# stevengj/nlopt

Measured on NVIDIA H100. Metric: ccsa_dual_evals_per_sec, higher is better.
Workload: dtype f64

## Files before the change

### nlopt_b200/csrc/ccsa_kernels.cuh

```cuda
#pragma once

#include <cuda_runtime.h>

#include <cstdint>

#include "dual_mma.hpp"
#include "pair_math.cuh"

namespace nb200 {

constexpr int kBlock = 256;
constexpr int kWarps = kBlock / 32;
constexpr int kVirtualShards = 8;
constexpr int kMaxParamM = 16;
constexpr int kMaxNV = 3 + kMaxParamM;
constexpr int kWideMaxM = 2048;

__device__ __forceinline__ double mulx(double a, double b) { return __dmul_rn(a, b); }
__device__ __forceinline__ double addx(double a, double b) { return __dadd_rn(a, b); }
__device__ __forceinline__ double subx(double a, double b) { return __dsub_rn(a, b); }
__device__ __forceinline__ double divx(double a, double b) { return __ddiv_rn(a, b); }

__device__ __forceinline__ unsigned long long nb_globaltimer()
{
// ... 1811 lines not shown
            } else {
                xc.x = ccsaq_point<MAXM, true>(mu, vx.x, vlb.x, vub.x, vs.x, vg.x, Ga, acc);
                xc.y = ccsaq_point<MAXM, true>(mu, vx.y, vlb.y, vub.y, vs.y, vg.y, Gb, acc);
            }
            if (store) st_stream(reinterpret_cast<double2 *>(a.xcur) + mt.p + sub * 32 + lane, xc);
        }
        if (mt.flags & 2u) {
            warp_fold<NV>(acc);
            double *srec = s_rec[parity];
            if (lane == 0) {
#pragma unroll
                for (int k = 0; k < NV; ++k) srec[sub * NV + k] = acc[k];
            }
            asm volatile("bar.sync 1, %0;" ::"r"(32 * kGroupWarps) : "memory");
            parity ^= 1;
            if (sub == 0) put_group_record<NV>(srec, a.grouptags, ngroups, mt.gl, sa.tag0 | my_gen, lane);
            NB_TR(if (sub == 0 && lane == 0 && my_gen < kTraceGens) { const unsigned long long t = nb_globaltimer(); unsigned long long *r = sa.trace + 16 * my_gen;
                      atomicMax(r + 3, ~t); atomicMax(r + 4, t); atomicAdd(r + 8, t - tr_s0); atomicAdd(r + 9, 1ull); tr_last = t; })
        }
    }
    if (threadIdx.x == 0) {
        s_stop = 1;
        while (!s_prod_done) __nanosleep(20);
        __threadfence_block();
        const unsigned long long issued = s_issued;
        unsigned long long done = consumed + 1;
        if (++st == STAGES) { st = 0; phase ^= 1u; }
        for (; done < issued; ++done) {
            mbar_wait(&s_full[st], phase);
            if (++st == STAGES) { st = 0; phase ^= 1u; }
        }
    }
    asm volatile("bar.sync 1, %0;" ::"r"(32 * kGroupWarps) : "memory");
}

constexpr int kPenaltyRowsPerLaunch = 16;
struct PenaltyCoefs {
    double c[kPenaltyRowsPerLaunch];
    int row[kPenaltyRowsPerLaunch];
    int count;
};
__global__ void __launch_bounds__(kBlock) penalty_axpy_kernel(double *__restrict__ g, const double *__restrict__ rows,
                                                               unsigned long long ld, unsigned long long n_local,
                                                               const __grid_constant__ PenaltyCoefs pc)
{
    const unsigned long long stride = (unsigned long long) gridDim.x * blockDim.x;
    for (unsigned long long j = (unsigned long long) blockIdx.x * blockDim.x + threadIdx.x; j < n_local; j += stride) {
        double v = g[j];
        for (int k = 0; k < pc.count; ++k) v = addx(v, mulx(pc.c[k], rows[(unsigned long long) pc.row[k] * ld + j]));
        g[j] = v;
    }
}

__global__ void __launch_bounds__(kBlock) negate_kernel(double *__restrict__ g, unsigned long long n_local)
{
    constexpr unsigned long long kSign = 0x8000000000000000ull;
    const unsigned long long pairs = n_local >> 1, stride = (unsigned long long) gridDim.x * blockDim.x;
    const unsigned long long t = (unsigned long long) blockIdx.x * blockDim.x + threadIdx.x;
    ulonglong2 *g2 = reinterpret_cast<ulonglong2 *>(g);
    for (unsigned long long p = t; p < pairs; p += stride) {
        ulonglong2 v = g2[p];
        v.x ^= kSign;
        v.y ^= kSign;
        g2[p] = v;
    }
    if ((n_local & 1) && t == 0) {
        unsigned long long *tail = reinterpret_cast<unsigned long long *>(g) + (n_local - 1);
        *tail ^= kSign;
    }
}

__global__ void publish_kernel(const double *all_vsums , int nv, int nvp, volatile double *out_host,
                               volatile unsigned long long *flag_host, unsigned long long seq)
{
    for (int k = threadIdx.x; k < nv; k += blockDim.x) {
        double s = all_vsums[k];
        for (int v = 1; v < kVirtualShards; ++v) s = addx(s, all_vsums[v * nvp + k]);
        out_host[k] = s;
    }
    __threadfence_system();
    __syncthreads();
    if (threadIdx.x == 0) {
        *flag_host = seq;
        __threadfence_system();
    }
}

constexpr int kBoxHaloLeft = 20, kBoxHaloRight = 21;
struct HaloArgs {
    double *x;
    unsigned long long n_local;
    unsigned long long right_cell;
    double *box[8];
    int rank, world;
    unsigned long long seq;
};
__global__ void halo_exchange_kernel(const __grid_constant__ HaloArgs a)
{
    const int lane = threadIdx.x;
    const int buf = (int) (a.seq & 1ull);
    const bool left = a.rank > 0, right = a.rank + 1 < a.world;
    if (lane == 0 && left)
        box_put(a.box[a.rank - 1] + 2ull * ((unsigned long long) buf * 8 * kBoxStride + kBoxHaloRight), a.x[0], a.seq);
    if (lane == 1 && right)
        box_put(a.box[a.rank + 1] + 2ull * ((unsigned long long) buf * 8 * kBoxStride + kBoxHaloLeft), a.x[a.n_local - 1], a.seq);
    if ((lane == 0 && left) || (lane == 1 && right)) {
        const double *mine = a.box[a.rank] + 2ull * ((unsigned long long) buf * 8 * kBoxStride + (lane == 0 ? kBoxHaloLeft : kBoxHaloRight));
        const unsigned long long t0 = nb_globaltimer();
        double v;
        bool ok;
        while (!(ok = box_get(mine, a.seq, &v)))
            if (nb_globaltimer() - t0 > 10000000000ull) break;
        if (!ok) v = __longlong_as_double(0x7ff8000000000000ll);
        if (lane == 0) a.x[-1] = v; else a.x[a.right_cell] = v;
    }
}
__global__ void halo_apply_kernel(double *x, unsigned long long right_cell, const double *edges, int rank, int world)
{
    if (threadIdx.x == 0 && rank > 0) x[-1] = edges[2 * (rank - 1) + 1];
    if (threadIdx.x == 1 && rank + 1 < world) x[right_cell] = edges[2 * (rank + 1)];
}
__global__ void halo_pack_kernel(const double *x, unsigned long long n_local, double *edges, int rank)
{
    if (threadIdx.x == 0) { edges[2 * rank] = x[0]; edges[2 * rank + 1] = x[n_local - 1]; }
}

__global__ void fill_kernel(double *dst, double value, unsigned long long n_local)
{
    for (unsigned long long j = blockIdx.x * (unsigned long long) blockDim.x + threadIdx.x; j < n_local;
         j += (unsigned long long) gridDim.x * blockDim.x)
        dst[j] = value;
}

__device__ __forceinline__ bool dev_isinf(double v) { return fabs(v) >= HUGE_VAL * 0.99 || isinf(v); }

__global__ void sigma_init_kernel(double *sigma, const double *lb, const double *ub, const double *sigma_init,
                                  double sigma_min, unsigned long long n_local, unsigned short *sidx)
{
    for (unsigned long long j = blockIdx.x * (unsigned long long) blockDim.x + threadIdx.x; j < n_local;
         j += (unsigned long long) gridDim.x * blockDim.x) {
        double s;
        if (sigma_init && sigma_init[j] > 0) s = sigma_init[j];
        else if (dev_isinf(ub[j]) || dev_isinf(lb[j])) s = 1.0;
        else s = mulx(0.5, subx(ub[j], lb[j]));
        sigma[j] = s > sigma_min ? s : sigma_min;
        if (sidx) sidx[j] = 1;
    }
}

struct EndOuterArgs {
    const double *xcur;
    double *xprev, *xprevprev, *sigma;
    const double *lb, *ub;
    const double *w;
    const double *xtol_abs;
    unsigned long long n_local, nchunks, chunk0;
    unsigned nseg_total, seg0, segs_per_vshard, local_vshards;
    double *partials, *vsums;
    unsigned *tickets;
    double *out_dev;
    volatile double *out_host;
    volatile unsigned long long *flag_host;
    unsigned long long seq;
    int publish_host, nvp;
    int update_sigma;
    double kappa;
    double sigma_min;
    unsigned short *sidx;
    const unsigned short *next;
    const double *pal;
};

__global__ void __launch_bounds__(kBlock) end_outer_kernel(const __grid_constant__ EndOuterArgs a)
{
    constexpr int NV = 4;
    __shared__ double s_red[kWarps * NV];
    __shared__ int s_flag;
    const unsigned seg = a.seg0 + blockIdx.x;
    unsigned long long p_lo, p_hi;
    group_pairs(a.nchunks, a.nseg_total, a.chunk0, seg, &p_lo, &p_hi);
    double acc[NV] = {0.0, 0.0, 0.0, 0.0};
    for (unsigned long long p = p_lo + threadIdx.x; p < p_hi; p += kBlock) {
#pragma unroll
        for (int h = 0; h < 2; ++h) {
            const unsigned long long j = 2 * p + h;
            if (j >= a.n_local) break;
            const double xc = a.xcur[j], xp = a.xprev[j];
            const double d = fabs(subx(xc, xp));
            if (a.w) {
                acc[0] = addx(acc[0], mulx(a.w[j], d));
                acc[1] = addx(acc[1], mulx(a.w[j], fabs(xc)));
            } else {
                acc[0] = addx(acc[0], d);
                acc[1] = addx(acc[1], fabs(xc));
            }
            if (a.xtol_abs && d >= a.xtol_abs[j]) acc[2] = addx(acc[2], 1.0);
            if (a.update_sigma) {
                const double xpp = a.xprevprev[j];
                const double osc = mulx(subx(xc, xp), subx(xp, xpp));
                const int br = osc < 0 ? 0 : (osc > 0 ? 1 : 2);
                const double s0 = a.sigma[j];
                double s = mulx(s0, br == 0 ? 0.7 : (br == 1 ? 1.2 : 1.0));
                const double lo = a.lb[j], hi = a.ub[j];
                if (!dev_isinf(hi) && !dev_isinf(lo)) {
                    const double range = subx(hi, lo);
                    const double top = mulx(10.0, range), bot = mulx(a.kappa, range);
                    s = s < top ? s : top;
                    s = s > bot ? s : bot;
                }
                s = s > a.sigma_min ? s : a.sigma_min;
                a.sigma[j] = s;
                if (a.sidx) {
                    const unsigned short i0 = a.sidx[j], t = a.next[3u * i0 + br];
                    a.sidx[j] = t;
                    if (__double_as_longlong(__ldg(a.pal + i0)) != __double_as_longlong(s0) ||
                        __double_as_longlong(__ldg(a.pal + t)) != __double_as_longlong(s))
                        acc[3] = addx(acc[3], 1.0);
                }
            }
            if (a.xprevprev) a.xprevprev[j] = xp;
            a.xprev[j] = xc;
        }
    }
    block_reduce_to<NV>(acc, s_red, a.partials + (unsigned long long) blockIdx.x * a.nvp);
    const unsigned vs_local = blockIdx.x / a.segs_per_vshard;
    if (!is_last_arrival(a.tickets + vs_local, a.segs_per_vshard, &s_flag)) return;
    acc[0] = acc[1] = acc[2] = acc[3] = 0.0;
    {
        const double *base = a.partials + (unsigned long long) vs_local * a.segs_per_vshard * a.nvp;
        for (unsigned sgi = threadIdx.x; sgi < a.segs_per_vshard; sgi += kBlock)
#pragma unroll
            for (int k = 0; k < NV; ++k) acc[k] = addx(acc[k], __ldcg(base + (unsigned long long) sgi * a.nvp + k));
    }
    block_reduce_to<NV>(acc, s_red, a.vsums + (unsigned long long) vs_local * a.nvp);
    if (!is_last_arrival(a.tickets + a.local_vshards, a.local_vshards, &s_flag)) return;
    if (threadIdx.x < NV) {
        if (a.publish_host) {
            double s = __ldcg(a.vsums + threadIdx.x);
            for (unsigned v = 1; v < a.local_vshards; ++v) s = addx(s, __ldcg(a.vsums + (unsigned long long) v * a.nvp + threadIdx.x));
            a.out_host[threadIdx.x] = s;
            __threadfence_system();
        } else {
            const unsigned v0 = a.seg0 / a.segs_per_vshard;
            for (unsigned v = 0; v < a.local_vshards; ++v)
                a.out_dev[(unsigned long long) (v0 + v) * a.nvp + threadIdx.x] = __ldcg(a.vsums + (unsigned long long) v * a.nvp + threadIdx.x);
        }
    }
    __syncthreads();
    if (threadIdx.x == 0) {
        for (unsigned v = 0; v <= a.local_vshards; ++v) a.tickets[v] = 0;
        if (a.publish_host) {
            *a.flag_host = a.seq;
            __threadfence_system();
        }
    }
}

}
```

### nlopt_b200/csrc/device_backend.cu

```cuda
#include "device_backend.hpp"

#include <chrono>
#include <cmath>
#include <cstdio>
#include <cstdlib>
#include <cstring>
#include <map>
#include <memory>
#include <mutex>
#include <string>
#include <vector>

#include "bounds_kernels.cuh"
#include "ccsa_kernels.cuh"
#include "comm.hpp"
#include "dual_mma.hpp"
#include "nlopt_object.hpp"
#include "synth.cuh"
#include "terms_kernels.cuh"

namespace nb200 {

namespace {

// ... 1328 lines not shown
    const bool tma_auto = solve_tma_ < 0 && scalar_bounds_ && (maxm == 4 || (maxm == 1 && operand_bytes <= ((size_t) 80 << 20)));
    size_t smem = 0;
    int block = 256;
    SolveKernel fn = nullptr;
    bool sb = false, si = false;
    if ((solve_tma_ > 0 || tma_auto) && full && !use_pol && (maxm == 1 || maxm == 2 || maxm == 4)) {
        sb = scalar_bounds_;
        si = sidx_valid_ && maxm == 4;
        const int bm = si ? kSigmaIndex : sb ? kScalarBounds : kBoundArrays;
        fn = variant_ == kMMA ? pick_solve_tma_kernel1<0>(bm, maxm, &smem) : pick_solve_tma_kernel1<1>(bm, maxm, &smem);
        block = kTmaBlock;
        NB_CUDA(cudaFuncSetAttribute((const void *) fn, cudaFuncAttributeMaxDynamicSharedMemorySize, (int) smem));
    } else if (solve_async_ >= 2 && !use_pol && maxm <= 8) {
        const int stages = solve_async_ >= 3 ? 3 : 2;
        fn = variant_ == kMMA ? pick_solve_async_kernel2<0>(maxm, full, stages) : pick_solve_async_kernel2<1>(maxm, full, stages);
        smem = (size_t) stages * (5 + (size_t) maxm) * kChunkBytes;
        NB_CUDA(cudaFuncSetAttribute((const void *) fn, cudaFuncAttributeMaxDynamicSharedMemorySize, (int) smem));
    } else {
        const bool roomy = solve_minb_ == 2 || (solve_minb_ != 3 && (long long) geo_.nseg_local + 1 <= 2ll * sm_count_);
        sb = scalar_bounds_ && !use_pol;
        fn = variant_ == kMMA ? pick_solve_kernel2<0>(maxm, full, use_pol, sb, roomy) : pick_solve_kernel2<1>(maxm, full, use_pol, sb, roomy);
    }
    int per_sm = 0;
    NB_CUDA(cudaOccupancyMaxActiveBlocksPerMultiprocessor(&per_sm, fn, block, smem));
    if (per_sm < 1) return fail("dual_solve_kernel does not fit on an SM");
    long long grid = (long long) per_sm * sm_count_;
    if (grid > (long long) geo_.nseg_local + 1) grid = (long long) geo_.nseg_local + 1;
    if (grid < 2) return fail("dual_solve_kernel needs two co-resident CTAs");

    NB_CUDA(cudaMemsetAsync(solve_state_, 0, offsetof(SolveState, pub), stream_));
    cudaEvent_t e0 = nullptr, e1 = nullptr;
    if (time_kernels_) {
        if (ev_used_ + 2 > ev_pool_.size()) {
            if (ev_pool_.size() >= 8192) drain_events();
            else
                for (int k = 0; k < 512; ++k) { cudaEvent_t e; cudaEventCreate(&e); ev_pool_.push_back(e); }
        }
        e0 = ev_pool_[ev_used_++];
        e1 = ev_pool_[ev_used_++];
        cudaEventRecord(e0, stream_);
    }
    void *params[] = {&sa};
    {
        cudaError_t le = cudaLaunchCooperativeKernel((const void *) fn, dim3((unsigned) grid), dim3((unsigned) block), params, smem, stream_);
        if (le != cudaSuccess) {
            cudaGetLastError();
            fused_solve_ok_ = false;
            if (ev_used_ >= 2 && time_kernels_) ev_used_ -= 2;
            return fail("cooperative launch of dual_solve_kernel", le);
        }
    }
    if (time_kernels_) cudaEventRecord(e1, stream_);
    ++stats_->kernel_launches;
    cand_in_x_ = false;
    ++x_epoch_;
    if (!wait_flag()) return false;
#ifdef NB200_TRACE
    if (const char *tf = std::getenv("NLOPT_B200_TRACE_FILE")) {
        static std::vector<unsigned long long> h(16 * kTraceGens);
        cudaStreamSynchronize(stream_);
        cudaMemcpy(h.data(), trace_buf, h.size() * sizeof(unsigned long long), cudaMemcpyDeviceToHost);
        std::string tfn = tf;
        if (Comm::instance().active()) tfn += ".r" + std::to_string(Comm::instance().rank);
        if (FILE *f = std::fopen(tfn.c_str(), "a")) {
            const unsigned long long t00 = ~h[1];
            std::fprintf(f, "solve n_local=%llu m=%u grid=%lld groups=%u cta_start_spread_ns=%llu first_publish_ns=%llu\n", (unsigned long long) geo_.n_local, m_, grid,
                         geo_.nseg_local, h[2] - t00, h[16] - t00);
            for (int g = 1; g < kTraceGens && h[16 * g]; ++g) {
                const unsigned long long *r = &h[16 * g];
                const unsigned long long p = r[0];
                std::fprintf(f, "  gen %d lastrec[%lld..%lld] parked[%lld..%lld] seen[%lld..%lld] recs[%lld..%lld] rank_done %lld totals %lld machine %lld next_pub %lld | mean_group_sweep %llu ns x %llu\n", g,
                             r[11] ? (long long) (~r[10] - p) : 0ll, r[11] ? (long long) (r[11] - p) : 0ll,
                             r[12] ? (long long) (~r[13] - p) : 0ll, r[12] ? (long long) (r[12] - p) : 0ll,
                             (long long) (~r[1] - p), (long long) (r[2] - p), (long long) (~r[3] - p), (long long) (r[4] - p),
                             (long long) (r[5] - p), (long long) (r[6] - p), (long long) (r[7] - p),
                             (long long) (h[16 * (g + 1)] ? h[16 * (g + 1)] - p : 0), r[9] ? r[8] / r[9] : 0ull, r[9]);
            }
            std::fclose(f);
        }
    }
#endif
    const long gens = (long) res_host_[kResCounts + 2];
    *ret = (int) res_host_[kResCounts + 1];
    *nevals = (long) res_host_[kResCounts];
    if (Comm::instance().active() && gens > 0) Comm::instance().advance_seq((unsigned long long) gens);
    if (*ret == kRetInvalid) return true;
    if (*ret == kRetFailure) return fail("the cross-rank exchange inside the dual solve timed out");
    count_operand_bytes(gens, sb, si, true);
    out->val = res_host_[0];
    out->gval = res_host_[1];
    out->wval = res_host_[2];
    for (unsigned i = 0; i < m_; ++i) {
        out->gc[i] = res_host_[3 + i];
        y[i] = res_host_[kResY + i];
    }
    return true;
}

void DeviceBackend::drain_events()
{
    if (!ev_used_) return;
    cudaStreamSynchronize(stream_);
    double ms = 0;
    for (size_t i = 0; i + 1 < ev_used_; i += 2) {
        float t = 0;
        if (cudaEventElapsedTime(&t, ev_pool_[i], ev_pool_[i + 1]) == cudaSuccess) ms += t;
    }
    stats_->seconds_dual_kernel += ms * 1e-3;
    ev_used_ = 0;
}

bool DeviceBackend::time_dual(const double *y, const DualScalars &sc, bool materialize, int iters, double *ms_avg)
{
    cudaEvent_t e0, e1;
    NB_CUDA(cudaEventCreate(&e0));
    NB_CUDA(cudaEventCreate(&e1));
    NB_CUDA(cudaEventRecord(e0, stream_));
    for (int it = 0; it < iters; ++it)
        if (!launch_dual(y, sc, materialize, false)) return false;
    NB_CUDA(cudaEventRecord(e1, stream_));
    NB_CUDA(cudaStreamSynchronize(stream_));
    float ms = 0;
    NB_CUDA(cudaEventElapsedTime(&ms, e0, e1));
    cudaEventDestroy(e0);
    cudaEventDestroy(e1);
    if (materialize) cand_in_x_ = false;
    *ms_avg = (double) ms / iters;
    return true;
}


void DeviceBackend::accept_candidate()
{
    std::swap(x_, xcur_);
    std::swap(g_, gcur_);
    std::swap(G_, Gcur_);
    cand_in_x_ = true;
    if (h_x_slot_ == (int) kCandidate && h_x_epoch_ == x_epoch_) h_x_slot_ = (int) kBase;
    if (h_xs_slot_ == (int) kCandidate && h_xs_epoch_ == x_epoch_) h_xs_slot_ = (int) kBase;
}

bool DeviceBackend::first_outer()
{
    NB_CUDA(cudaMemcpyAsync(xprev_, xcur_view(), geo_.ld * sizeof(double), cudaMemcpyDeviceToDevice, stream_));
    return true;
}

bool DeviceBackend::end_outer(unsigned k, double sigma_min, double *dnorm, double *xnorm, bool *all_below_abs)
{
    EndOuterArgs a;
    std::memset(&a, 0, sizeof a);
    a.xcur = xcur_view();
    a.xprev = xprev_; a.xprevprev = xprevprev_; a.sigma = sigma_;
    a.lb = lb_; a.ub = ub_;
    a.update_sigma = k > 1;
    a.kappa = variant_ == kMMA ? 0.01 : 1e-8;
    a.sigma_min = sigma_min;
    if (a.update_sigma && sidx_valid_) {
        sidx_valid_ = sigma_min == sidx_sigma_min_ && palette_.step();
        if (sidx_valid_ && !upload_palette()) return false;
        if (sidx_valid_) { a.sidx = sidx_; a.next = next_; a.pal = pal_; }
    }
    if (!end_outer_pass(a, dnorm, xnorm, all_below_abs)) return false;
    if (out_host_[3] != 0.0) {
        stats_->sigma_index_mismatches += (long long) out_host_[3];
        sidx_valid_ = false;
    }
    stats_->sigma_palette = sidx_valid_ ? (long long) palette_.val.size() : 0;
    return true;
}

bool DeviceBackend::end_outer_pass(EndOuterArgs &a, double *dnorm, double *xnorm, bool *all_below_abs)
{
    a.w = w_dev_; a.xtol_abs = xtol_abs_dev_;
    a.n_local = geo_.n_local; a.nchunks = geo_.nchunks; a.chunk0 = geo_.chunk0;
    a.nseg_total = geo_.S; a.seg0 = geo_.seg0; a.segs_per_vshard = geo_.P; a.local_vshards = geo_.local_vshards;
    a.partials = partials_; a.vsums = vsums_; a.tickets = tickets_; a.out_dev = out_dev_;
    a.out_host = out_host_; a.flag_host = flag_host_;
    a.seq = seq_ = Comm::instance().active() ? Comm::instance().next_seq() : seq_ + 1;
    a.publish_host = Comm::instance().active() ? 0 : 1;
    a.nvp = kEndNvp;
    end_outer_kernel<<<(int) geo_.nseg_local, kBlock, 0, stream_>>>(a);
    ++stats_->kernel_launches;
    NB_CUDA(cudaGetLastError());
    if (!a.publish_host) {
        if (Comm::instance().all_gather_inplace(out_dev_, (size_t) geo_.local_vshards * kEndNvp, stream_, &err_)) return false;
        publish_kernel<<<1, 32, 0, stream_>>>(out_dev_, 4, kEndNvp, out_host_, flag_host_, a.seq);
        ++stats_->kernel_launches;
        NB_CUDA(cudaGetLastError());
    }
    if (!wait_flag()) return false;
    *dnorm = out_host_[0];
    *xnorm = out_host_[1];
    *all_below_abs = out_host_[2] == 0.0;
    return true;
}

bool DeviceBackend::stop_x_keep(double *dnorm, double *xnorm, bool *all_below_abs)
{
    EndOuterArgs a;
    std::memset(&a, 0, sizeof a);
    a.xcur = x_;
    a.xprev = xprev_;
    return end_outer_pass(a, dnorm, xnorm, all_below_abs);
}

int DeviceBackend::ranks() const { return Comm::instance().active() ? Comm::instance().world : 1; }

bool DeviceBackend::fetch_x(double *x_out)
{
    drain_events();
    if (cfg_.values_only) {
        NB_CUDA(cudaMemcpyAsync(x_out, xprev_, geo_.n_local * sizeof(double), cfg_.x_dev ? cudaMemcpyDeviceToDevice : cudaMemcpyDeviceToHost, stream_));
        NB_CUDA(cudaStreamSynchronize(stream_));
        if (!cfg_.x_dev) stats_->d2h_bytes += geo_.n_local * sizeof(double);
        return true;
    }
    if (cfg_.x_dev && x_out == cfg_.x_dev) {
        NB_CUDA(cudaMemcpyAsync(x_out, x_, geo_.n_local * sizeof(double), cudaMemcpyDeviceToDevice, stream_));
        NB_CUDA(cudaStreamSynchronize(stream_));
        return true;
    }
    Comm &comm = Comm::instance();
    if (!comm.active()) {
        NB_CUDA(cudaMemcpyAsync(x_out, x_, geo_.n_local * sizeof(double), cudaMemcpyDeviceToHost, stream_));
        NB_CUDA(cudaStreamSynchronize(stream_));
        stats_->d2h_bytes += geo_.n_local * sizeof(double);
        return true;
    }
    if (!h_x_) NB_CUDA(cached_host_alloc(&h_x_, (size_t) geo_.n * sizeof(double)));
    if (!xfull_dev_) NB_CUDA(cached_malloc(&xfull_dev_, (size_t) comm.world * shard_cap_ * sizeof(double)));
    h_x_slot_ = -1;
    if (!host_x_for(kBase)) return false;
    std::memcpy(x_out, h_x_view_, (size_t) geo_.n * sizeof(double));
    return true;
}


double *DeviceBackend::array(const char *which)
{
    const std::string w = which;
    if (w == "x") return x_;
    if (w == "xcur") return xcur_view();
    if (w == "xprev") return xprev_;
    if (w == "xprevprev") return xprevprev_;
    if (w == "lb") return lb_;
    if (w == "ub") return ub_;
    if (w == "sigma") return sigma_;
    if (w == "grad_f") return g_;
    if (w == "grad_f_cur") return gcur_;
    return nullptr;
}

bool DeviceBackend::upload(const char *which, const double *host)
{
    double *dst = array(which);
    if (std::string(which) == "xcur") { dst = xcur_; cand_in_x_ = false; }
    if (!dst) return fail(std::string("unknown array ") + which);
    if (dst == sigma_) sidx_valid_ = false;
    NB_CUDA(cudaMemcpyAsync(dst, host + geo_.j0, geo_.n_local * sizeof(double), cudaMemcpyHostToDevice, stream_));
    NB_CUDA(cudaStreamSynchronize(stream_));
    return true;
}

bool DeviceBackend::upload_grad_c(const double *host)
{
    if (!m_) return true;
    NB_CUDA(cudaMemcpy2DAsync(G_, geo_.ld * sizeof(double), host + geo_.j0, (size_t) geo_.n * sizeof(double),
                              geo_.n_local * sizeof(double), m_, cudaMemcpyHostToDevice, stream_));
    NB_CUDA(cudaStreamSynchronize(stream_));
    return true;
}

bool DeviceBackend::download(const char *which, double *host)
{
    const std::string w = which;
    if (w == "grad_c") {
        if (!m_) return true;
        NB_CUDA(cudaMemcpy2DAsync(host + geo_.j0, (size_t) geo_.n * sizeof(double), G_, geo_.ld * sizeof(double),
                                  geo_.n_local * sizeof(double), m_, cudaMemcpyDeviceToHost, stream_));
        NB_CUDA(cudaStreamSynchronize(stream_));
        return true;
    }
    double *src = array(which);
    if (!src) return fail(std::string("unknown array ") + which);
    NB_CUDA(cudaMemcpyAsync(host + geo_.j0, src, geo_.n_local * sizeof(double), cudaMemcpyDeviceToHost, stream_));
    NB_CUDA(cudaStreamSynchronize(stream_));
    return true;
}

bool DeviceBackend::fill_synthetic(unsigned long long seed)
{
    SynthArgs a;
    a.x = x_; a.lb = lb_; a.ub = ub_; a.sigma = sigma_; a.g = g_; a.G = G_;
    a.ld = geo_.ld; a.n_local = geo_.n_local; a.j0 = geo_.j0; a.seed = seed; a.m = (int) m_;
    synth_fill_kernel<<<grid_for(geo_.n_local, sm_count_), kBlock, 0, stream_>>>(a);
    NB_CUDA(cudaGetLastError());
    NB_CUDA(cudaStreamSynchronize(stream_));
    cand_in_x_ = true;
    return true;
}

bool DeviceBackend::configure(const char *key, long long value)
{
    const std::string k = key;
    if (k == "time_kernels") { time_kernels_ = value != 0; return true; }
    if (k == "kernel_cfg") { kernel_cfg_ = (int) value; return true; }
    if (k == "ctas_per_sm") { ctas_per_sm_ = (int) value; return true; }
    if (k == "fused_solve") { fused_solve_ok_ = value != 0; return true; }
    if (k == "solve_tma") { solve_tma_ = (int) value; return true; }
    if (k == "solve_async") { solve_async_ = (int) value; return true; }
    if (k == "solve_minb") { solve_minb_ = (int) value; return true; }
    if (k == "l2_keep_mb") {
        l2_keep_bytes_ = value <= 0 ? 0 : (size_t) value << 20;
        int maxp = 0;
        if (cudaDeviceGetAttribute(&maxp, cudaDevAttrMaxPersistingL2CacheSize, device_) == cudaSuccess && maxp > 0) {
            size_t want = l2_keep_bytes_ < (size_t) maxp ? l2_keep_bytes_ : (size_t) maxp;
            cudaDeviceSetLimit(cudaLimitPersistingL2CacheSize, want);
            cudaGetLastError();
        }
        return true;
    }
    if (k == "pmax" || k == "target_chunks" || k == "fill_div" || k == "group_base" || k == "geometry_rule" || k == "group_min_chunks") {
        if (value < 1 && k != "geometry_rule") return fail("bad value");
        if (k == "pmax") pmax_ = (unsigned) value;
        else if (k == "target_chunks") target_chunks_ = (unsigned) value;
        else if (k == "group_base") Geometry::group_base() = (unsigned) value;
        else if (k == "group_min_chunks") Geometry::min_group_chunks() = (unsigned) value;
        else if (k == "geometry_rule") Geometry::rule() = (int) value;
        else Geometry::fill_div() = (unsigned) value;
        if (pool_) {
            Geometry g2 = Geometry::make(geo_.n, geo_.world, geo_.rank, target_chunks_, pmax_);
            if (g2.ld != geo_.ld || g2.j0 != geo_.j0)
                return fail("changing the segment geometry of a sharded, allocated problem is not supported");
            geo_ = g2;
            return alloc_workspace();
        }
        return true;
    }
    return fail(std::string("unknown key ") + key);
}

long long DeviceBackend::query(const char *key) const
{
    const std::string k = key;
    if (k == "kernel_ns") {
        const_cast<DeviceBackend *>(this)->drain_events();
        return (long long) (stats_->seconds_dual_kernel * 1e9);
    }
    if (k == "segments") return geo_.S;
    if (k == "segments_local") return geo_.nseg_local;
    if (k == "P") return geo_.P;
    if (k == "n_local") return (long long) geo_.n_local;
    if (k == "j0") return (long long) geo_.j0;
    if (k == "ld") return (long long) geo_.ld;
    if (k == "launches") return stats_->kernel_launches;
    if (k == "maxm") return pick_maxm((int) m_);
// ... 399 lines not shown
```

### nlopt_b200/csrc/device_backend.hpp

```cpp
#pragma once

#include <cuda_runtime.h>

#include <string>
#include <vector>

#include "backend_factory.hpp"
#include "geometry.hpp"
#include "sigma_palette.hpp"

#ifndef NB200_SIGMA_INDEX_MIN_MB
#define NB200_SIGMA_INDEX_MIN_MB 50
#endif

namespace nb200 {

class DeviceBackend : public Backend {
public:
    DeviceBackend();
    ~DeviceBackend() override;

    bool setup(const BackendConfig &cfg);
    bool setup_raw(Variant v, unsigned n, unsigned m);

    unsigned n() const override { return (unsigned) geo_.n; }
    unsigned m() const override { return m_; }
    unsigned num_constraint_objects() const override { return (unsigned) cfg_.constraints.size(); }
    unsigned constraint_dim(unsigned ic) const override { return cfg_.constraints[ic].m; }
    bool init_sigma(double sigma_min) override;
    bool eval_objective(Slot slot, bool want_grad, double *value) override;
    bool eval_constraint(Slot slot, unsigned ic, unsigned row0, bool want_grad, double *values) override;
    bool finish_evals(double *fvalue, double *cvalues) override;
    bool agree_any(bool local) override;
    bool enqueue_df2(const FuncSpec &fs, Slot slot, double *grad_dst, unsigned index);
    bool reduce_terms(const FuncSpec &fs, const double *xs, double *grad_dst, double *vsums);
    bool ensure_halo(Slot slot);
    bool eval_sharded(const FuncSpec &fs, Slot slot, double *grad_dst, unsigned index, double *value);
    bool eval_user_objective(Slot slot, bool want_grad, double *value);
    bool negate_gradient(double *g);
    bool push_rows_to(double *dst, unsigned rows, const double *host_grad);
    bool eval_penalty_objective(Slot slot, bool want_grad, double *value);
    bool dual_eval(const double *y, const DualScalars &sc, bool materialize, DualSums *out) override;
    bool supports_dual_solve() const override;
    bool dual_solve(double *y, const double *lo, const double *hi, const double *stop6, const DualScalars &sc, DualSums *out,
                    int *ret, long *nevals) override;
    void accept_candidate() override;
    bool first_outer() override;
    bool end_outer(unsigned k, double sigma_min, double *dnorm, double *xnorm, bool *all_below_abs) override;
    bool fetch_x(double *x_out) override;
    double *point_device() override { return cfg_.values_only ? x_ : nullptr; }
    void point_moved() override { ++x_epoch_; }
    bool stop_x_keep(double *dnorm, double *xnorm, bool *all_below_abs) override;
    int ranks() const override;
    const std::string &error() const override { return err_; }
    double seconds_in_callbacks() const override { return cb_seconds_; }

    bool upload(const char *which, const double *host);
    bool upload_grad_c(const double *host_rowmajor_m_by_n);
    bool download(const char *which, double *host);
    bool fill_synthetic(unsigned long long seed);
    bool sigma_init_from(const double *sigma_init_host, double sigma_min);
    bool set_norm_arrays(const double *x_weights_host, const double *xtol_abs_host);
    bool time_dual(const double *y, const DualScalars &sc, bool materialize, int iters, double *ms_avg);
    bool configure(const char *key, long long value) override;
    long long query(const char *key) const;
    const Geometry &geometry() const { return geo_; }
    bool is_mma() const { return variant_ == kMMA; }

private:
    bool fail(const char *what, cudaError_t e);
    bool fail(const std::string &what);
    bool alloc_state();
    void free_state();
    bool alloc_workspace();
    double *array(const char *which);
    double *xcur_view() { return cand_in_x_ ? x_ : xcur_; }
    void fill_dual_args(struct DualArgs &a, const double *y, const DualScalars &sc);
    bool launch_dual(const double *y, const DualScalars &sc, bool store, bool wait);
    bool end_outer_pass(struct EndOuterArgs &a, double *dnorm, double *xnorm, bool *all_below_abs);
    unsigned l2_keep_mask() const;
    void count_operand_bytes(long long evals, bool sb, bool si, bool store);
    bool upload_palette();
    bool sigma_index_runs() const;
    bool wait_flag();
    bool host_x_for(Slot slot);
    bool push_grad_rows(Slot slot, int row0, unsigned rows, bool is_objective, const double *host_grad);
    double *staging(unsigned rows);
    struct Owned { void *p; size_t bytes; bool pinned; };
    std::vector<Owned> owned_;
    bool small_dev(void **p, size_t bytes);
    bool small_pinned(void **p, size_t bytes);
    void release_small(void *p);

    BackendConfig cfg_;
    Variant variant_ = kMMA;
    unsigned m_ = 0;
    Geometry geo_;
    unsigned target_chunks_ = kDefaultTargetChunks, pmax_ = kDefaultPmax;
    int device_ = 0;
    int sm_count_ = 132, ctas_per_sm_ = 0;
    void *solve_state_ = nullptr;
    double *res_host_ = nullptr;
    double *grouptags_ = nullptr;
    unsigned long long eval_tag_ = 0;
    double *wide_dev_ = nullptr;
    std::vector<double> wide_host_;
    size_t l2_keep_bytes_ = 0;
    int solve_tma_ = -1;
    int solve_async_ = 0;
    int solve_minb_ = 0;
    size_t out_rec_ = 0;
    unsigned long long solve_launch_id_ = 0;
    bool fused_solve_ok_ = true;
    bool scalar_bounds_ = false;
    double lb_u_ = 0.0, ub_u_ = 0.0;
    bool sidx_valid_ = false;
    unsigned short *sidx_ = nullptr, *next_ = nullptr;
    double *pal_ = nullptr;
    double *pal_pinned_ = nullptr;
    unsigned short *next_pinned_ = nullptr;
    SigmaPalette palette_;
    size_t pal_uploaded_ = 0, rows_uploaded_ = 0;
    double sidx_sigma_min_ = 0.0;
    int kernel_cfg_ = -1;

    double *pool_ = nullptr;
    size_t pool_bytes_ = 0;
    double *x_ = nullptr, *xcur_ = nullptr, *xprev_ = nullptr, *xprevprev_ = nullptr, *lb_ = nullptr, *ub_ = nullptr,
           *sigma_ = nullptr, *g_ = nullptr, *gcur_ = nullptr, *G_ = nullptr, *Gcur_ = nullptr;
    double *w_dev_ = nullptr, *xtol_abs_dev_ = nullptr;
    bool cand_in_x_ = true;

    double *partials_ = nullptr, *vsums_ = nullptr, *out_dev_ = nullptr;
    unsigned *tickets_ = nullptr;
    double *out_host_ = nullptr;
    unsigned long long *flag_host_ = nullptr;
    unsigned long long seq_ = 0;
    int nvp_ = 24;

    double *h_x_ = nullptr;
    double *h_x_view_ = nullptr;
    double *h_grad_[2] = {nullptr, nullptr};
    size_t h_grad_cap_ = 0;
    int h_grad_next_ = 0;
    cudaEvent_t h_grad_done_[2] = {nullptr, nullptr};
    double *h_xs_ = nullptr, *h_gs_[2] = {nullptr, nullptr};
    cudaEvent_t h_gs_done_[2] = {nullptr, nullptr};
    int h_gs_next_ = 0, h_xs_slot_ = -1;
    unsigned long long h_xs_epoch_ = 0;
    double *xfull_dev_ = nullptr;
    double *pen_rows_ = nullptr;
    unsigned pen_total_ = 0;
    double *scalar_dev_ = nullptr;
    std::vector<double> pend_val_;
    std::vector<char> pend_set_;
    bool pend_any_ = false;
    size_t scalar_cap_ = 0;
    double *vs2_dev_ = nullptr, *vs2_host_ = nullptr;
    size_t vs2_cap_ = 0;
    std::vector<const FuncSpec *> pend2_;
    bool pend2_any_ = false;
    unsigned terms_rows_ = 0;
    double *terms_ = nullptr, *terms_part_ = nullptr;
    nlopt_b200_shard shard_{};
    double *halo_edges_ = nullptr;
    const double *halo_ptr_ = nullptr;
    unsigned long long halo_epoch_ = 0;
    size_t shard_cap_ = 0;
    unsigned long long x_epoch_ = 1, h_x_epoch_ = 0;
    int h_x_slot_ = -1;

    cudaStream_t stream_ = nullptr, copy_stream_ = nullptr;

    bool time_kernels_ = false;
    std::vector<cudaEvent_t> ev_pool_;
    size_t ev_used_ = 0;
    void drain_events();

    std::string err_;
    double cb_seconds_ = 0;
    nlopt_b200_stats local_stats_{};
    nlopt_b200_stats *stats_ = &local_stats_;
    unsigned max_cdim_ = 1;
};

void release_cached_blocks();

}
```

Before: 5716.

## Vectorize end_outer loads/stores, use scalar bounds, rotate xprev buffers

The end-of-outer-iteration kernel now loads and stores element pairs with double2/ushort2 vector accesses. When bounds are uniform it uses scalar bound values instead of reading the lb/ub arrays. It also writes xcur into the xprevprev buffer and swaps the xprev/xprevprev pointers on the host, which saves one array write per element. This cuts global memory traffic in a bandwidth-bound kernel. The risks are alignment assumptions for the vector accesses and correctness of the buffer rotation when xprevprev is null or the first pass differs.

After: 5717, median of 6. Within noise of the previous version (+0.0%).

```diff
diff --git a/nlopt_b200/csrc/ccsa_kernels.cuh b/nlopt_b200/csrc/ccsa_kernels.cuh
--- a/nlopt_b200/csrc/ccsa_kernels.cuh
+++ b/nlopt_b200/csrc/ccsa_kernels.cuh
@@ -1987,6 +1987,8 @@
     const double *xcur;
     double *xprev, *xprevprev, *sigma;
     const double *lb, *ub;
+    double lb_u, ub_u;
+    int rotate;
     const double *w;
     const double *xtol_abs;
     unsigned long long n_local, nchunks, chunk0;
@@ -2006,6 +2008,29 @@
     const double *pal;
 };
 
+template <class T, class T2>
+__device__ __forceinline__ void ld_pair(T (&v)[2], const T *row, unsigned long long j, bool full)
+{
+    if (full) {
+        const T2 t = *reinterpret_cast<const T2 *>(row + j);
+        v[0] = t.x;
+        v[1] = t.y;
+    } else
+        v[0] = row[j];
+}
+template <class T, class T2>
+__device__ __forceinline__ void st_pair(T *row, unsigned long long j, const T (&v)[2], bool full)
+{
+    if (full) {
+        T2 t;
+        t.x = v[0];
+        t.y = v[1];
+        *reinterpret_cast<T2 *>(row + j) = t;
+    } else
+        row[j] = v[0];
+}
+
+template <bool SB = false>
 __global__ void __launch_bounds__(kBlock) end_outer_kernel(const __grid_constant__ EndOuterArgs a)
 {
     constexpr int NV = 4;
@@ -2016,45 +2041,65 @@
     group_pairs(a.nchunks, a.nseg_total, a.chunk0, seg, &p_lo, &p_hi);
     double acc[NV] = {0.0, 0.0, 0.0, 0.0};
     for (unsigned long long p = p_lo + threadIdx.x; p < p_hi; p += kBlock) {
+        const unsigned long long j0 = 2 * p;
+        if (j0 >= a.n_local) break;
+        const bool full = j0 + 1 < a.n_local;
+        const int nh = full ? 2 : 1;
+        double xc[2] = {0.0, 0.0}, xp[2] = {0.0, 0.0}, xpp[2] = {0.0, 0.0}, s0[2] = {0.0, 0.0};
+        double lo[2] = {a.lb_u, a.lb_u}, hi[2] = {a.ub_u, a.ub_u}, s[2] = {0.0, 0.0};
+        unsigned short i0[2] = {0, 0}, t[2] = {0, 0};
+        ld_pair<double, double2>(xc, a.xcur, j0, full);
+        ld_pair<double, double2>(xp, a.xprev, j0, full);
+        if (a.update_sigma) {
+            ld_pair<double, double2>(xpp, a.xprevprev, j0, full);
+            ld_pair<double, double2>(s0, a.sigma, j0, full);
+            if (!SB) {
+                ld_pair<double, double2>(lo, a.lb, j0, full);
+                ld_pair<double, double2>(hi, a.ub, j0, full);
+            }
+            if (a.sidx) ld_pair<unsigned short, ushort2>(i0, a.sidx, j0, full);
+        }
 #pragma unroll
         for (int h = 0; h < 2; ++h) {
-            const unsigned long long j = 2 * p + h;
-            if (j >= a.n_local) break;
-            const double xc = a.xcur[j], xp = a.xprev[j];
-            const double d = fabs(subx(xc, xp));
+            if (h >= nh) break;
+            const unsigned long long j = j0 + h;
+            const double d = fabs(subx(xc[h], xp[h]));
             if (a.w) {
                 acc[0] = addx(acc[0], mulx(a.w[j], d));
-                acc[1] = addx(acc[1], mulx(a.w[j], fabs(xc)));
+                acc[1] = addx(acc[1], mulx(a.w[j], fabs(xc[h])));
             } else {
                 acc[0] = addx(acc[0], d);
-                acc[1] = addx(acc[1], fabs(xc));
+                acc[1] = addx(acc[1], fabs(xc[h]));
             }
             if (a.xtol_abs && d >= a.xtol_abs[j]) acc[2] = addx(acc[2], 1.0);
             if (a.update_sigma) {
-                const double xpp = a.xprevprev[j];
-                const double osc = mulx(subx(xc, xp), subx(xp, xpp));
+                const double osc = mulx(subx(xc[h], xp[h]), subx(xp[h], xpp[h]));
                 const int br = osc < 0 ? 0 : (osc > 0 ? 1 : 2);
-                const double s0 = a.sigma[j];
-                double s = mulx(s0, br == 0 ? 0.7 : (br == 1 ? 1.2 : 1.0));
-                const double lo = a.lb[j], hi = a.ub[j];
-                if (!dev_isinf(hi) && !dev_isinf(lo)) {
-                    const double range = subx(hi, lo);
+                double sh = mulx(s0[h], br == 0 ? 0.7 : (br == 1 ? 1.2 : 1.0));
+                if (!dev_isinf(hi[h]) && !dev_isinf(lo[h])) {
+                    const double range = subx(hi[h], lo[h]);
                     const double top = mulx(10.0, range), bot = mulx(a.kappa, range);
-                    s = s < top ? s : top;
-                    s = s > bot ? s : bot;
+                    sh = sh < top ? sh : top;
+                    sh = sh > bot ? sh : bot;
                 }
-                s = s > a.sigma_min ? s : a.sigma_min;
-                a.sigma[j] = s;
+                s[h] = sh > a.sigma_min ? sh : a.sigma_min;
                 if (a.sidx) {
-                    const unsigned short i0 = a.sidx[j], t = a.next[3u * i0 + br];
-                    a.sidx[j] = t;
-                    if (__double_as_longlong(__ldg(a.pal + i0)) != __double_as_longlong(s0) ||
-                        __double_as_longlong(__ldg(a.pal + t)) != __double_as_longlong(s))
+                    t[h] = a.next[3u * i0[h] + br];
+                    if (__double_as_longlong(__ldg(a.pal + i0[h])) != __double_as_longlong(s0[h]) ||
+                        __double_as_longlong(__ldg(a.pal + t[h])) != __double_as_longlong(s[h]))
                         acc[3] = addx(acc[3], 1.0);
                 }
             }
-            if (a.xprevprev) a.xprevprev[j] = xp;
-            a.xprev[j] = xc;
+        }
+        if (a.update_sigma) {
+            st_pair<double, double2>(a.sigma, j0, s, full);
+            if (a.sidx) st_pair<unsigned short, ushort2>(a.sidx, j0, t, full);
+        }
+        if (a.rotate)
+            st_pair<double, double2>(a.xprevprev, j0, xc, full);
+        else {
+            if (a.xprevprev) st_pair<double, double2>(a.xprevprev, j0, xp, full);
+            st_pair<double, double2>(a.xprev, j0, xc, full);
         }
     }
     block_reduce_to<NV>(acc, s_red, a.partials + (unsigned long long) blockIdx.x * a.nvp);
diff --git a/nlopt_b200/csrc/device_backend.cu b/nlopt_b200/csrc/device_backend.cu
--- a/nlopt_b200/csrc/device_backend.cu
+++ b/nlopt_b200/csrc/device_backend.cu
@@ -1504,7 +1504,9 @@
     std::memset(&a, 0, sizeof a);
     a.xcur = xcur_view();
     a.xprev = xprev_; a.xprevprev = xprevprev_; a.sigma = sigma_;
-    a.lb = lb_; a.ub = ub_;
+    a.rotate = 1;
+    if (scalar_bounds_) { a.lb_u = lb_u_; a.ub_u = ub_u_; }
+    else { a.lb = lb_; a.ub = ub_; }
     a.update_sigma = k > 1;
     a.kappa = variant_ == kMMA ? 0.01 : 1e-8;
     a.sigma_min = sigma_min;
@@ -1513,7 +1515,9 @@
         if (sidx_valid_ && !upload_palette()) return false;
         if (sidx_valid_) { a.sidx = sidx_; a.next = next_; a.pal = pal_; }
     }
-    if (!end_outer_pass(a, dnorm, xnorm, all_below_abs)) return false;
+    const bool ok = end_outer_pass(a, dnorm, xnorm, all_below_abs, scalar_bounds_);
+    std::swap(xprev_, xprevprev_);
+    if (!ok) return false;
     if (out_host_[3] != 0.0) {
         stats_->sigma_index_mismatches += (long long) out_host_[3];
         sidx_valid_ = false;
@@ -1522,7 +1526,7 @@
     return true;
 }
 
-bool DeviceBackend::end_outer_pass(EndOuterArgs &a, double *dnorm, double *xnorm, bool *all_below_abs)
+bool DeviceBackend::end_outer_pass(EndOuterArgs &a, double *dnorm, double *xnorm, bool *all_below_abs, bool sb)
 {
     a.w = w_dev_; a.xtol_abs = xtol_abs_dev_;
     a.n_local = geo_.n_local; a.nchunks = geo_.nchunks; a.chunk0 = geo_.chunk0;
@@ -1532,7 +1536,8 @@
     a.seq = seq_ = Comm::instance().active() ? Comm::instance().next_seq() : seq_ + 1;
     a.publish_host = Comm::instance().active() ? 0 : 1;
     a.nvp = kEndNvp;
-    end_outer_kernel<<<(int) geo_.nseg_local, kBlock, 0, stream_>>>(a);
+    if (sb) end_outer_kernel<true><<<(int) geo_.nseg_local, kBlock, 0, stream_>>>(a);
+    else end_outer_kernel<false><<<(int) geo_.nseg_local, kBlock, 0, stream_>>>(a);
     ++stats_->kernel_launches;
     NB_CUDA(cudaGetLastError());
     if (!a.publish_host) {
@@ -1554,7 +1559,7 @@
     std::memset(&a, 0, sizeof a);
     a.xcur = x_;
     a.xprev = xprev_;
-    return end_outer_pass(a, dnorm, xnorm, all_below_abs);
+    return end_outer_pass(a, dnorm, xnorm, all_below_abs, false);
 }
 
 int DeviceBackend::ranks() const { return Comm::instance().active() ? Comm::instance().world : 1; }
diff --git a/nlopt_b200/csrc/device_backend.hpp b/nlopt_b200/csrc/device_backend.hpp
--- a/nlopt_b200/csrc/device_backend.hpp
+++ b/nlopt_b200/csrc/device_backend.hpp
@@ -77,7 +77,7 @@
     double *xcur_view() { return cand_in_x_ ? x_ : xcur_; }
     void fill_dual_args(struct DualArgs &a, const double *y, const DualScalars &sc);
     bool launch_dual(const double *y, const DualScalars &sc, bool store, bool wait);
-    bool end_outer_pass(struct EndOuterArgs &a, double *dnorm, double *xnorm, bool *all_below_abs);
+    bool end_outer_pass(struct EndOuterArgs &a, double *dnorm, double *xnorm, bool *all_below_abs, bool sb);
     unsigned l2_keep_mask() const;
     void count_operand_bytes(long long evals, bool sb, bool si, bool store);
     bool upload_palette();
```
